# JuliaGaussianProcesses/ApproximateGPs.jl

Hardware: AMD Instinct MI355X
Metric: SVGP ELBO evals/sec at N=1e6, M=1024 (higher is better)
Workload: dtype f64

## Files before the change

### approximategps.jl_amd/csrc/device_common.hpp

```cpp
#pragma once
#include <hip/hip_runtime.h>
#include <type_traits>
#include <utility>

#include "diag.hpp"
#include <stdint.h>

#include <mutex>
#include <string>
#include <vector>

namespace svgp {

inline std::string& note_text() { static thread_local std::string s; return s; }
inline void leave_note(const std::string& s) {
  if (note_text().size() < 2048) note_text() += (note_text().empty() ? "" : "; ") + s;
}
inline std::string take_note() {
  std::string s;
  s.swap(note_text());
  return s;
}

inline void set_max_lds(const void* fn, hipFuncAttribute attr, int bytes) {
  struct Entry { const void* fn; int dev; int bytes; };
  static std::mutex mu;
  static std::vector<Entry> seen;
  int dev = 0;
  (void)hipGetDevice(&dev);
  std::lock_guard<std::mutex> g(mu);
  for (Entry& e : seen)
    if (e.fn == fn && e.dev == dev) {
      if (bytes <= e.bytes) return;
      if (hipFuncSetAttribute(fn, attr, bytes) == hipSuccess) e.bytes = bytes;
      else leave_note("hipFuncSetAttribute(" + std::to_string(bytes) + " bytes of LDS) failed");
      return;
    }
  const hipError_t err = hipFuncSetAttribute(fn, attr, bytes);
  if (err == hipSuccess) seen.push_back(Entry{fn, dev, bytes});
  else leave_note(std::string("hipFuncSetAttribute(") + std::to_string(bytes) + " bytes of LDS) failed: " + hipGetErrorString(err));
}

constexpr int kWave = 64;
constexpr int kThreads = 512;
constexpr int k256 = 256;
constexpr int kNB = 128;

template <typename T>
struct Mfma16;

template <>
struct Mfma16<double> {
  using acc_t = double __attribute__((ext_vector_type(4)));
  static __device__ __forceinline__ acc_t mma(double a, double b, acc_t c) {
    return __builtin_amdgcn_mfma_f64_16x16x4f64(a, b, c, 0, 0, 0);
  }
  static __device__ __forceinline__ int row(int lane, int r) { return (lane >> 4) + 4 * r; }
};

template <>
struct Mfma16<float> {
  using acc_t = float __attribute__((ext_vector_type(4)));
  static __device__ __forceinline__ acc_t mma(float a, float b, acc_t c) {
    return __builtin_amdgcn_mfma_f32_16x16x4f32(a, b, c, 0, 0, 0);
  }
  static __device__ __forceinline__ int row(int lane, int r) { return (lane >> 4) * 4 + r; }
};

template <typename T>
struct Vec16 {
  static constexpr int N = 16 / sizeof(T);
  using type = T __attribute__((ext_vector_type(16 / sizeof(T))));
};

enum : int { KSE = 0, KM32 = 1, KM52 = 2 };

__device__ __forceinline__ double kexp(double v) {
  const double n = rint(v * 1.4426950408889634074);
  double r = fma(n, -6.93147180369123816490e-01, v);
  r = fma(n, -1.90821492927058770002e-10, r);
  double p = 1.6059043836821613e-10;
  p = fma(p, r, 2.08767569878681e-09);
  p = fma(p, r, 2.505210838544172e-08);
  p = fma(p, r, 2.755731922398589e-07);
  p = fma(p, r, 2.7557319223985893e-06);
  p = fma(p, r, 2.48015873015873e-05);
  p = fma(p, r, 1.984126984126984e-04);
  p = fma(p, r, 1.3888888888888889e-03);
  p = fma(p, r, 8.333333333333333e-03);
  p = fma(p, r, 4.1666666666666664e-02);
  p = fma(p, r, 1.6666666666666666e-01);
  p = fma(p, r, 0.5);
  p = fma(p, r, 1.0);
  p = fma(p, r, 1.0);
  return ldexp(p, int(n));
}
__device__ __forceinline__ float kexp(float v) {
  const float hi = v * 1.44269504088896341f;
  const float lo = fmaf(v, 1.44269504088896341f, -hi) + v * 1.92596299112661746e-8f;
  const float e = __builtin_amdgcn_exp2f(hi);
  return fmaf(e, lo * 0.693147180559945309f, e);
}
__device__ __forceinline__ double kexp_tab(double v, const double* __restrict__ tab) {
  const double nd = rint(v * 92.332482616893658);
  const int n = int(nd);
  double r = fma(nd, -1.08304246932675596327e-02, v);
  r = fma(nd, -2.98158582698529328128e-12, r);
  const double t = tab[n & 63];
  double p = fma(r, 8.333333333333333e-03, 4.1666666666666664e-02);
  p = fma(p, r, 1.6666666666666666e-01);
  p = fma(p, r, 0.5);
  p = fma(p, r, 1.0);
  p *= r;
  return ldexp(fma(t, p, t), n >> 6);
}

__device__ __forceinline__ double ksqrt(double v) { return sqrt(v); }
__device__ __forceinline__ float ksqrt(float v) { return __builtin_amdgcn_sqrtf(v); }

template <typename T>
__device__ __forceinline__ T kappa(int family, T r2, T variance) {
  if (family == KSE) return variance * kexp(T(-0.5) * r2);
  T r = ksqrt(r2);
  if (family == KM32) {
    T s = T(1.7320508075688772935) * r;
    return variance * (T(1) + s) * kexp(-s);
  }
  T s = T(2.2360679774997896964) * r;
  return variance * (T(1) + s + T(5.0 / 3.0) * r2) * kexp(-s);
}

template <typename T>
__device__ __forceinline__ T kappa_2g(int family, T r2, T variance, T kval) {
  if (family == KSE) return -kval;
  T r = ksqrt(r2);
  if (family == KM32) {
    T s = T(1.7320508075688772935) * r;
    return (T(-3) * variance) * kexp(-s);
  }
  T s = T(2.2360679774997896964) * r;
  return (T(-5.0 / 3.0) * variance) * ((T(1) + s) * kexp(-s));
}

template <typename T, int NT, int BK, int NTHR = kThreads, int PAD = 16>
struct TileGemm {
  static constexpr int NB = kNB;
  static constexpr int WR = 2, WC = NTHR / 128;
  static constexpr int MI = NB / WR / 16;
  static constexpr int NJ = NT / WC / 16;
  static constexpr int PLD = NB + PAD;
  static constexpr int QLD = NT + PAD;
  static constexpr int VEC = Vec16<T>::N;
  using V = typename Vec16<T>::type;
  using acc_t = typename Mfma16<T>::acc_t;

  static constexpr int P_TPR = NB / VEC;
  static constexpr int P_RPP = NTHR / P_TPR;
  static constexpr int P_PASSES = BK / P_RPP;
  static constexpr int Q_TPR = NT / VEC;
  static constexpr int Q_RPP = NTHR / Q_TPR;
  static constexpr int Q_PASSES = (BK / Q_RPP) > 0 ? (BK / Q_RPP) : 1;
  static_assert(BK % P_RPP == 0, "BK must be a multiple of the P rows per pass");
  static_assert(BK % Q_RPP == 0 || Q_RPP % BK == 0, "BK and the Q rows per pass must divide one another");
  static constexpr bool Q_PARTIAL = Q_RPP > BK;

  static constexpr int P_TILE = BK * PLD;
  static constexpr int Q_TILE = BK * QLD;
  static constexpr int STAGE = P_TILE + Q_TILE;
  static constexpr size_t LDS_BYTES = 2 * size_t(STAGE) * sizeof(T);

  struct Acc {
    acc_t v[MI][NJ];
    __device__ __forceinline__ void zero() {
#pragma unroll
      for (int i = 0; i < MI; ++i)
#pragma unroll
        for (int j = 0; j < NJ; ++j) v[i][j] = acc_t{0, 0, 0, 0};
    }
  };

  struct PRegs { V v[P_PASSES]; };
  struct QRegs { V v[Q_PASSES]; };

  struct POff { uint32_t o[P_PASSES]; };
  struct QOff { uint32_t o[Q_PASSES]; };
  static __device__ __forceinline__ POff p_offsets(int64_t ld) {
    POff r;
    const int t = threadIdx.x;
    const int kk0 = t / P_TPR, c = (t % P_TPR) * VEC;
#pragma unroll
    for (int p = 0; p < P_PASSES; ++p) r.o[p] = uint32_t((int64_t(kk0 + p * P_RPP) * ld + c) * sizeof(T));
    return r;
  }
  static __device__ __forceinline__ QOff q_offsets(int64_t ld) {
    QOff r;
    const int t = threadIdx.x;
    const int kk0 = t / Q_TPR, c = (t % Q_TPR) * VEC;
#pragma unroll
    for (int p = 0; p < Q_PASSES; ++p) r.o[p] = uint32_t((int64_t(kk0 + p * Q_RPP) * ld + c) * sizeof(T));
    return r;
  }
  static __device__ __forceinline__ void load_p(PRegs& r, const T* __restrict__ src, const POff& off) {
    if constexpr (diag::ablate<1>) {
      asm volatile("" : "+v"(r.v[0]));
      return;
    }
    const char* base = reinterpret_cast<const char*>(src);
#pragma unroll
    for (int p = 0; p < P_PASSES; ++p) r.v[p] = *reinterpret_cast<const V*>(base + off.o[p]);
  }
  static __device__ __forceinline__ void store_p(const PRegs& r, T* __restrict__ Ps) {
    const int t = threadIdx.x;
    const int kk0 = t / P_TPR, c = (t % P_TPR) * VEC;
#pragma unroll
    for (int p = 0; p < P_PASSES; ++p) *reinterpret_cast<V*>(Ps + (kk0 + p * P_RPP) * PLD + c) = r.v[p];
  }
#ifndef SVGP_DMA_P
#define SVGP_DMA_P 1
#endif
#ifndef SVGP_DMA_ASM
#define SVGP_DMA_ASM 1
#endif
  static constexpr int NW = NTHR / 64;
  static constexpr bool kDmaP = SVGP_DMA_P && (NB * sizeof(T) == 1024) && (BK % NW == 0);
  static constexpr int D_ROWS = BK / NW;
  struct DOff { uint32_t o[D_ROWS]; };
  static __device__ __forceinline__ DOff d_offsets(int64_t ld) {
    DOff r;
    const int lane = threadIdx.x & 63, wave = threadIdx.x >> 6;
#pragma unroll
    for (int q = 0; q < D_ROWS; ++q) r.o[q] = uint32_t((int64_t(wave + q * NW) * ld + lane * VEC) * sizeof(T));
    return r;
  }
  static __device__ __forceinline__ void glds16(const void* sbase, uint32_t voff, const T* lds) {
#if SVGP_DMA_ASM
    const uint32_t l = uint32_t(uintptr_t((__attribute__((address_space(3))) T*)(lds)));
    asm volatile("s_mov_b32 m0, %0\n\tglobal_load_lds_dwordx4 %1, %2" ::"s"(l), "v"(voff), "s"(sbase) : "memory");
#else
    __builtin_amdgcn_global_load_lds((const __attribute__((address_space(1))) void*)(reinterpret_cast<const char*>(sbase) + voff),
                                     (__attribute__((address_space(3))) void*)(lds), 16, 0, 0);
#endif
  }
  static __device__ __forceinline__ void dma_p(const T* __restrict__ src, const DOff& off, T* __restrict__ Ps) {
    if constexpr (diag::ablate<1>) return;
    const int wv = __builtin_amdgcn_readfirstlane(int(threadIdx.x >> 6));
#pragma unroll
    for (int q = 0; q < D_ROWS; ++q) glds16(src, off.o[q], Ps + (wv + q * NW) * PLD);
  }
  static __device__ __forceinline__ void load_q(QRegs& r, const T* __restrict__ src, const QOff& off) {
    if constexpr (diag::ablate<2>) {
      asm volatile("" : "+v"(r.v[0]));
      return;
    }
    const char* base = reinterpret_cast<const char*>(src);
    if (Q_PARTIAL && int(threadIdx.x) >= BK * Q_TPR) return;
#pragma unroll
    for (int p = 0; p < Q_PASSES; ++p) r.v[p] = *reinterpret_cast<const V*>(base + off.o[p]);
  }
  static __device__ __forceinline__ void load_q_trans(QRegs& r, const T* __restrict__ src, int64_t ld) {
    const int t = threadIdx.x;
    const int kk0 = t / Q_TPR, c = (t % Q_TPR) * VEC;
#pragma unroll
    for (int p = 0; p < Q_PASSES; ++p)
#pragma unroll
      for (int e = 0; e < VEC; ++e) r.v[p][e] = src[int64_t(c + e) * ld + (kk0 + p * Q_RPP)];
  }
  static __device__ __forceinline__ void store_q(const QRegs& r, T* __restrict__ Qs) {
    const int t = threadIdx.x;
    const int kk0 = t / Q_TPR, c = (t % Q_TPR) * VEC;
    if (Q_PARTIAL && t >= BK * Q_TPR) return;
#pragma unroll
    for (int p = 0; p < Q_PASSES; ++p) *reinterpret_cast<V*>(Qs + (kk0 + p * Q_RPP) * QLD + c) = r.v[p];
  }
  static __device__ __forceinline__ void q_coord(int p, int& kk, int& c) {
    const int t = threadIdx.x;
    kk = t / Q_TPR + p * Q_RPP;
    c = (t % Q_TPR) * VEC;
  }

  struct Frag {
    T a[MI], b[NJ];
  };
  static __device__ __forceinline__ int wave_row() { return __builtin_amdgcn_readfirstlane(int(threadIdx.x >> 6)) / WC; }
  static __device__ __forceinline__ int frag_a_off() {
    const int lane = threadIdx.x & 63, wave = threadIdx.x >> 6;
    return (lane >> 4) * PLD + (wave / WC) * 16 + (lane & 15);
  }
  static __device__ __forceinline__ int frag_b_off() {
    const int lane = threadIdx.x & 63, wave = threadIdx.x >> 6;
    return (lane >> 4) * QLD + (wave % WC) * (NJ * 16) + (lane & 15);
  }
  template <int BUF, int KSLAB, int ILO = 0, int IHI = MI - 1>
  static __device__ __forceinline__ void load_frag(Frag& f, const T* __restrict__ fa, const T* __restrict__ fb) {
#pragma unroll
    for (int i = 0; i < MI; ++i)
      if (i >= ILO && i <= IHI) f.a[i] = fa[BUF * STAGE + KSLAB * 4 * PLD + i * 32];
    if (ILO <= IHI) {
#pragma unroll
      for (int j = 0; j < NJ; ++j) f.b[j] = fb[BUF * STAGE + KSLAB * 4 * QLD + j * 16];
    }
  }
  template <int ILO = 0, int IHI = MI - 1>
  static __device__ __forceinline__ void mma_frag(Acc& acc, const Frag& f) {
#pragma unroll
    for (int i = 0; i < MI; ++i)
      if (i >= ILO && i <= IHI) {
#pragma unroll
        for (int j = 0; j < NJ; ++j) acc.v[i][j] = Mfma16<T>::mma(f.a[i], f.b[j], acc.v[i][j]);
      }
  }

  static __device__ __forceinline__ int acc_row(int i, int r) {
    const int lane = threadIdx.x & 63, wave = threadIdx.x >> 6;
    return (2 * i + wave / WC) * 16 + Mfma16<T>::row(lane, r);
  }
  static __device__ __forceinline__ int acc_col(int j) {
    const int lane = threadIdx.x & 63, wave = threadIdx.x >> 6;
    return (wave % WC) * (NJ * 16) + j * 16 + (lane & 15);
  }

  static constexpr int kLoopPrologueBarriers = 1, kLoopClosingBarriers = 1;
  static constexpr int kAsyncPrologueBarriers = 1, kAsyncClosingBarriers = 1;
  static constexpr int loop_barrier_count(int nsteps) { return nsteps <= 0 ? 0 : kLoopPrologueBarriers + nsteps + kLoopClosingBarriers; }
  static constexpr int async_barrier_count(int nsteps) { return nsteps <= 0 ? 0 : kAsyncPrologueBarriers + (nsteps - 1) + kAsyncClosingBarriers; }

  template <int BUF, int ILO, int IHI, typename QLoad>
  static __device__ __forceinline__ void step(Acc& acc, Frag (&f)[2], PRegs& pr, QRegs& qr, const T* __restrict__ Pbase,
                                              int64_t pstride, const POff& poff, const DOff& doff, int t, int nsteps,
                                              QLoad& qload, T* __restrict__ smem, const T* __restrict__ fa,
                                              const T* __restrict__ fb) {
    constexpr int KS = BK / 4;
    static_assert(KS % 2 == 0, "the fragment ping-pong needs an even number of k-slabs per step");
    const bool more = (t + 1 < nsteps);
#pragma unroll
    for (int ks = 0; ks + 1 < KS; ++ks) {
      if (ks == 0) load_frag<BUF, 1, ILO, IHI>(f[1], fa, fb);
      if (ks == 1) load_frag<BUF, 2, ILO, IHI>(f[0], fa, fb);
      if (ks == 2) load_frag<BUF, 3, ILO, IHI>(f[1], fa, fb);
      if (ks == 3) load_frag<BUF, 4 < KS ? 4 : 0, ILO, IHI>(f[0], fa, fb);
      if (ks == 4) load_frag<BUF, 5 < KS ? 5 : 0, ILO, IHI>(f[1], fa, fb);
      if (ks == 5) load_frag<BUF, 6 < KS ? 6 : 0, ILO, IHI>(f[0], fa, fb);
      if (ks == 6) load_frag<BUF, 7 < KS ? 7 : 0, ILO, IHI>(f[1], fa, fb);
      mma_frag<ILO, IHI>(acc, f[ks & 1]);
    }
    if (more) {
      T* Pn = smem + (BUF ^ 1) * STAGE;
      if constexpr (!kDmaP) store_p(pr, Pn);
      store_q(qr, Pn + P_TILE);
    }
    __syncthreads();
    if (more) {
      load_frag<BUF ^ 1, 0>(f[0], fa, fb);
      if (t + 2 < nsteps) {
        if constexpr (kDmaP) {
          qload(t + 2, qr);
          dma_p(Pbase + int64_t(t + 2) * pstride, doff, smem + BUF * STAGE);
        } else {
          load_p(pr, Pbase + int64_t(t + 2) * pstride, poff);
          qload(t + 2, qr);
        }
      }
    }
    mma_frag<ILO, IHI>(acc, f[(KS - 1) & 1]);
  }

#define SVGP_DSTEP(B, LO, HI, TT) step<B, LO, HI>(acc, f, pr, qr, Pbase, pstride, poff, doff, (TT), nsteps, qload, smem, fa, fb)

  template <typename QLoad>
  static __device__ __forceinline__ void loop(Acc& acc, const T* __restrict__ Pbase, int64_t ldp, int nsteps,
                                              QLoad&& qload, T* __restrict__ smem) {
    loop_tri<0>(acc, Pbase, ldp, nsteps, qload, smem);
  }

  template <int TRI, typename QLoad>
  static __device__ __forceinline__ void loop_tri(Acc& acc, const T* __restrict__ Pbase, int64_t ldp, int nsteps,
                                                  QLoad&& qload, T* __restrict__ smem) {
    if (nsteps <= 0) return;
    static_assert(BK <= 32, "step() enumerates at most 8 k-slabs");
    constexpr int ND = NB / BK;
    static_assert(TRI == 0 || (ND == 8 && MI == 4), "triangular steps are written out for BK = 16, 128-row panels");
    const POff poff = p_offsets(ldp);
    const DOff doff = d_offsets(ldp);
    const int64_t pstride = int64_t(BK) * ldp;
    const T* fa = smem + frag_a_off();
    const T* fb = smem + P_TILE + frag_b_off();
    PRegs pr;
    QRegs qr;
    if constexpr (kDmaP) {
      qload(0, qr);
      dma_p(Pbase, doff, smem);
    } else {
      load_p(pr, Pbase, poff);
      qload(0, qr);
      store_p(pr, smem);
    }
    store_q(qr, smem + P_TILE);
    __syncthreads();
    if (nsteps > 1) {
      if constexpr (kDmaP) {
        qload(1, qr);
        dma_p(Pbase + pstride, doff, smem + STAGE);
      } else {
        load_p(pr, Pbase + pstride, poff);
        qload(1, qr);
      }
    }
    Frag f[2];
    load_frag<0, 0>(f[0], fa, fb);
    int t = 0;
    if (TRI < 0) {
      SVGP_DSTEP(0, 0, 0, 0); SVGP_DSTEP(1, 0, 0, 1); SVGP_DSTEP(0, 0, 1, 2); SVGP_DSTEP(1, 0, 1, 3);
      SVGP_DSTEP(0, 0, 2, 4); SVGP_DSTEP(1, 0, 2, 5); SVGP_DSTEP(0, 0, 3, 6); SVGP_DSTEP(1, 0, 3, 7);
      t = ND;
    }
    const int nreg = (TRI > 0) ? nsteps - ND : nsteps;
    for (; t + 1 < nreg; t += 2) {
      step<0, 0, MI - 1>(acc, f, pr, qr, Pbase, pstride, poff, doff, t, nsteps, qload, smem, fa, fb);
      step<1, 0, MI - 1>(acc, f, pr, qr, Pbase, pstride, poff, doff, t + 1, nsteps, qload, smem, fa, fb);
    }
    if (t < nreg) step<0, 0, MI - 1>(acc, f, pr, qr, Pbase, pstride, poff, doff, t, nsteps, qload, smem, fa, fb);
    if (TRI > 0) {
      SVGP_DSTEP(0, 0, 3, nreg + 0); SVGP_DSTEP(1, 0, 3, nreg + 1); SVGP_DSTEP(0, 1, 3, nreg + 2); SVGP_DSTEP(1, 1, 3, nreg + 3);
      SVGP_DSTEP(0, 2, 3, nreg + 4); SVGP_DSTEP(1, 2, 3, nreg + 5); SVGP_DSTEP(0, 3, 3, nreg + 6); SVGP_DSTEP(1, 3, 3, nreg + 7);
    }
    __syncthreads();
  }
#undef SVGP_DSTEP

  static constexpr bool kPairP = (NB * sizeof(T) == 512);
#ifndef SVGP_ASYNC_QUAD
#define SVGP_ASYNC_QUAD 1
#endif
  static constexpr bool kRowQ = (NT * sizeof(T) == 1024);
  static constexpr int QR = kRowQ ? 1 : ((NT * sizeof(T) == 256) ? 4 : 2);
  static constexpr bool kAsync = (SVGP_DMA_P != 0) && (NB * sizeof(T) == 1024 || kPairP) &&
                                 (NT * sizeof(T) == 512 || (SVGP_ASYNC_QUAD && NT * sizeof(T) == 256) || (kRowQ && NTHR == 512)) &&
                                 BK == 16 && (NTHR == 256 || (kRowQ && NTHR == 512)) && NJ % 2 == 0;
  static constexpr int NBUF = 3;
  static constexpr int QPP = kRowQ ? QLD : QR * NT;
  static constexpr int QA_TILE = (BK / QR) * QPP;
  static constexpr int QSLAB = (4 / QR) * QPP;
  static constexpr int PPP = 2 * NB;
  static constexpr int PA_TILE = kPairP ? (BK / 2) * PPP : P_TILE;
  static constexpr int DQ = (BK / QR) / NW;
  static constexpr int DP = kPairP ? (BK / 2) / NW : BK / NW;
  static constexpr int DMA_PER_TILE = DP + DQ;
  static constexpr size_t ASYNC_LDS_BYTES = size_t(NBUF) * (PA_TILE + QA_TILE) * sizeof(T);
  static constexpr int W_TILE = 256 / int(sizeof(T));
  static constexpr size_t ASYNC_W_LDS_BYTES = ASYNC_LDS_BYTES + size_t(NBUF) * 256;
  static constexpr size_t MAX_LDS_BYTES = (kAsync && ASYNC_LDS_BYTES > LDS_BYTES) ? ASYNC_LDS_BYTES : LDS_BYTES;

  struct AOff { uint32_t p[DP]; uint32_t q[DQ]; };
  static __device__ __forceinline__ AOff a_offsets(int64_t ldp, int64_t ldq) {
    AOff r;
    const int lane = threadIdx.x & 63, wave = threadIdx.x >> 6;
    const int row = lane >> 5, slot = (lane & 31) * VEC;
#pragma unroll
    for (int q = 0; q < DP; ++q) {
      if constexpr (kPairP) r.p[q] = uint32_t((int64_t((wave + q * NW) * 2 + row) * ldp + (slot ^ (row * 16))) * sizeof(T));
      else r.p[q] = uint32_t((int64_t(wave + q * NW) * ldp + lane * VEC) * sizeof(T));
    }
    constexpr int LPR = 64 / QR;
    const int qrow = lane / LPR, qslot = (lane % LPR) * VEC;
#pragma unroll
    for (int q = 0; q < DQ; ++q)
      r.q[q] = uint32_t((int64_t((wave + q * NW) * QR + qrow) * ldq + (qslot ^ (qrow * 16))) * sizeof(T));
    return r;
  }
  static __device__ __forceinline__ int wave_index() { return __builtin_amdgcn_readfirstlane(int(threadIdx.x >> 6)); }
  static __device__ __forceinline__ void dma_tile(const T* __restrict__ psrc, const T* __restrict__ qsrc, const AOff& off,
                                                  T* __restrict__ Pb, T* __restrict__ Qb) {
    const int wv = wave_index();
// ... 364 lines not shown
```

### approximategps.jl_amd/csrc/strip.hip

```cpp
#define SVGP_DIAG_TU_STRIP
#include "device_common.hpp"
#include "kernels.hpp"
#include "knobs.hpp"
#include "lik.hpp"

#ifndef SVGP_ASYNC
#define SVGP_ASYNC 1
#endif
#ifndef SVGP_TRI
#define SVGP_TRI 3
#endif

#include <cstdlib>
#include <type_traits>

namespace svgp {

namespace {

#ifndef SVGP_PREGEN_EXPTAB
#define SVGP_PREGEN_EXPTAB 1
#endif
template <typename T, int NT, int NTHR, int F, int DL>
__device__ __forceinline__ void pregen_mfma(const T* __restrict__ xs, const T* __restrict__ zs, int d, int64_t Mp, int64_t M,
                                            double variance_d, T* __restrict__ work, const double* __restrict__ exptab = nullptr) {
  constexpr int KS = DL / 4, JT = NT / 16, NW = NTHR / 64;
  constexpr bool XREG = (DL <= 16);
  using M16 = Mfma16<T>;
  using acc_t = typename M16::acc_t;
  const int lane = threadIdx.x & 63, wave = threadIdx.x >> 6, l15 = lane & 15, g = lane >> 4;
  const T variance = T(variance_d);
  const T c1 = (F == KSE) ? T(-0.5) : T(1);
  const T c0 = (F == KSE) ? T(log(variance_d)) : T(0);
  const T ascale = (F == KSE) ? T(1) : T(-2);
  T xb[XREG ? JT : 1][XREG ? KS : 1], xn[JT];
  const T* __restrict__ xl = xs + g * NT + l15;
#pragma unroll
  for (int jt = 0; jt < JT; ++jt) {
    T s = T(0);
#pragma unroll
    for (int q = 0; q < KS; ++q) {
      const T v = xl[(4 * q) * NT + jt * 16];
      if constexpr (XREG) xb[jt][q] = v;
      s = fma(v, v, s);
    }
    s += __shfl_xor(s, 16);
    s += __shfl_xor(s, 32);
    xn[jt] = fma(c1, s, c0);
  }
  for (int kb = wave; kb < int(Mp / 16); kb += NW) {
    const int64_t k0 = int64_t(kb) * 16;
    const bool inside = __builtin_amdgcn_readfirstlane(int(k0 + 16 <= M)) != 0;
    T za[KS];
    T s = T(0);
#pragma unroll
    for (int q = 0; q < KS; ++q) {
      const int f = 4 * q + g;
      const T v = (f < d) ? zs[int64_t(f) * Mp + k0 + l15] : T(0);
      za[q] = ascale * v;
      s = fma(v, v, s);
    }
    s += __shfl_xor(s, 16);
    s += __shfl_xor(s, 32);
    s *= c1;
    T zn[4];
#pragma unroll
    for (int r = 0; r < 4; ++r) zn[r] = __shfl(s, M16::row(lane, r));
#pragma unroll
    for (int jt = 0; jt < JT; ++jt) {
      acc_t acc;
#pragma unroll
      for (int r = 0; r < 4; ++r) acc[r] = xn[jt] + zn[r];
      if constexpr (XREG) {
#pragma unroll
        for (int q = 0; q < KS; ++q) acc = M16::mma(za[q], xb[jt][q], acc);
      } else {
        acc_t acc2 = {0, 0, 0, 0};
        __builtin_amdgcn_sched_barrier(0);
#pragma unroll
        for (int q = 0; q < KS; q += 2) {
          acc = M16::mma(za[q], xl[(4 * q) * NT + jt * 16], acc);
          acc2 = M16::mma(za[q + 1], xl[(4 * q + 4) * NT + jt * 16], acc2);
        }
#pragma unroll
        for (int r = 0; r < 4; ++r) acc[r] += acc2[r];
      }
      T out[4];
#pragma unroll
      for (int r = 0; r < 4; ++r) {
        const T v = acc[r];
        if constexpr (SVGP_PREGEN_EXPTAB && F == KSE && sizeof(T) == 8) out[r] = T(kexp_tab(double(v > c0 ? c0 : v), exptab));
        else out[r] = (F == KSE) ? kexp(v > c0 ? c0 : v) : kappa<T>(F, v < T(0) ? T(0) : v, variance);
      }
      if (inside) {
#pragma unroll
        for (int r = 0; r < 4; ++r) work[(k0 + M16::row(lane, r)) * NT + jt * 16 + l15] = out[r];
      } else {
#pragma unroll
        for (int r = 0; r < 4; ++r) {
          const int64_t k = k0 + M16::row(lane, r);
          work[k * NT + jt * 16 + l15] = (k < M) ? out[r] : T(0);
        }
        asm volatile("" ::: "memory");
      }
    }
  }
}


template <typename G, typename T, int NT, int NTHR>
__device__ __forceinline__ void store_tile_point_major(const typename G::Acc& acc, T* __restrict__ smem, T* __restrict__ out,
                                                       int64_t c0, int64_t Mp, int row0) {
  constexpr int HC = NT < 64 ? NT : 64, RS = G::NB + (sizeof(T) == 8 ? 4 : 8), VEC = G::VEC, CPR = G::NB / VEC;
  using V = typename G::V;
  static_assert(size_t(HC) * RS * sizeof(T) <= ((SVGP_ASYNC && G::kAsync) ? G::ASYNC_LDS_BYTES : G::LDS_BYTES),
                "the transposition tile must fit the staging buffers");
#pragma unroll
  for (int p = 0; p < NT / HC; ++p) {
#pragma unroll
    for (int j = 0; j < G::NJ; ++j) {
      const int col = G::acc_col(j);
      if (col / HC == p) {
#pragma unroll
        for (int i = 0; i < G::MI; ++i)
#pragma unroll
          for (int r = 0; r < 4; ++r) smem[(col % HC) * RS + G::acc_row(i, r)] = acc.v[i][j][r];
      }
    }
    __syncthreads();
    for (int e = threadIdx.x; e < HC * CPR; e += NTHR) {
      const int col = e / CPR, rv = (e % CPR) * VEC;
      *reinterpret_cast<V*>(out + (c0 + p * HC + col) * Mp + row0 + rv) = *reinterpret_cast<const V*>(smem + col * RS + rv);
    }
    __syncthreads();
  }
}

#ifndef SVGP_STRIP_PRIO
#define SVGP_STRIP_PRIO 1
#endif
template <bool ON>
__device__ __forceinline__ void strip_prio(int strips_done) {
  if constexpr (ON && SVGP_STRIP_PRIO != 0) {
    if ((strips_done + (blockIdx.x >= gridDim.x / 2 ? 1 : 0)) & 1) __builtin_amdgcn_s_setprio(0);
    else __builtin_amdgcn_s_setprio(1);
  }
}

struct PointGrads { double e, gmu, gv, gs2; };
__device__ __noinline__ PointGrads strip_point_grads(LikParams lp, double mu, double v, double yv, double scale) {
  double a = 0.0, b = 0.0, gs2 = 0.0;
  expected_loglik_grad_point(lp, mu, v, yv, a, b, gs2);
  PointGrads r;
  r.e = expected_loglik_point(lp, mu, v, yv, log(lp.sigma2));
  r.gmu = a * scale;
  r.gv = b * scale;
  r.gs2 = gs2 * scale;
  return r;
}

template <typename T, int NT, int BK, int NTHR, int MINW = 2, int PAD = 16, bool GRAD = false, bool BIGD = false, bool SEG = false>
__global__ void __launch_bounds__(NTHR, MINW) strip_kernel(StripArgs a, int64_t nstrips) {
  using G = TileGemm<T, NT, BK, NTHR, PAD>;
  using Acc = typename G::Acc;
  using QRegs = typename G::QRegs;
  constexpr int NB = G::NB, MI = G::MI, NJ = G::NJ, VEC = G::VEC;

  extern __shared__ __attribute__((aligned(16))) unsigned char smem_raw[];
  T* smem = reinterpret_cast<T*>(smem_raw);
  T* xs = smem;
  const int pre_dl = BIGD ? (a.kp.d <= 32 ? 32 : 64) : (a.kp.d <= 8 ? 8 : a.kp.d <= 16 ? 16 : 0);
  const int dl = pre_dl ? pre_dl : a.kp.d;

  const T* __restrict__ Tm = static_cast<const T*>(a.T);
  const T* __restrict__ U = static_cast<const T*>(a.U);
  const T* __restrict__ zs = static_cast<const T*>(a.zs);
  const T* __restrict__ mp = static_cast<const T*>(a.mp);
  const T* __restrict__ x = static_cast<const T*>(a.x);
  const T* __restrict__ invl = static_cast<const T*>(a.kp.invl);
  const int64_t Mp = a.Mp, M = a.M;
  const int d = a.kp.d, family = a.kp.family;
  const T variance = T(a.kp.variance);
  const int nP = int(Mp / NB);
  T* __restrict__ work = static_cast<T*>(a.work) + int64_t(blockIdx.x) * Mp * NT;
  T* __restrict__ workK = (GRAD && !diag::ablate<256>) ? static_cast<T*>(a.work) + (int64_t(gridDim.x) + blockIdx.x) * Mp * NT : work;
  const int tid = threadIdx.x, lane = tid & 63;
  const typename G::QOff qoff = G::q_offsets(NT);

  __shared__ unsigned next_strip;
#if SVGP_PREGEN_EXPTAB
  __shared__ double s_exptab[64];
  if (sizeof(T) == 8 && threadIdx.x < 64) s_exptab[threadIdx.x] = exp2(double(threadIdx.x) * 0.015625);
  const double* exptab = s_exptab;
#else
  const double* exptab = nullptr;
#endif
  SVGP_SSTAMP_KERNEL_BEGIN();
  [[maybe_unused]] int prio_strips = 0;
  [[maybe_unused]] int part = 0, nsplit = 1;
  if constexpr (SEG) {
    if (a.seg_split > 1) { nsplit = a.seg_split; part = int(blockIdx.x / nstrips); }
  }
  for (int64_t strip = (nsplit > 1) ? int64_t(blockIdx.x % nstrips) : int64_t(blockIdx.x); strip < nstrips;) {
    if constexpr (SEG) {
      work = static_cast<T*>(a.work) + strip * Mp * NT;
      workK = GRAD ? static_cast<T*>(a.work) + (nstrips + strip) * Mp * NT : work;
    }
    SVGP_SSTAMP_STRIP_BEGIN();
    SVGP_SSTAMP(0);
    strip_prio<GRAD && !SEG>(prio_strips++);
    const int64_t c0 = strip * NT;
    if constexpr (SEG) { if (tid == 0) next_strip = unsigned(strip + gridDim.x); }
    else if (tid == 0) next_strip = gridDim.x + atomicAdd(a.counter, 1u);
    const int64_t last = a.off + a.len - 1;
    const bool do_pregen = !SEG || (a.seg_flags & kSegPregen);
    if (do_pregen)
    for (int e = tid; e < dl * NT; e += NTHR) {
      const int f = e / NT, c = e % NT;
      int64_t g = a.off + c0 + c;
      g = g > last ? last : g;
      xs[e] = (f < d) ? x[int64_t(f) * a.ldx + g] * invl[f] : T(0);
    }
    __syncthreads();
    if (do_pregen) {
      auto pregen = [&](auto fam) {
        constexpr int F = decltype(fam)::value;
        using V = typename G::V;
        constexpr int CPR = NT / VEC;
        for (int e = tid; e < int(Mp) * CPR; e += NTHR) {
          const int k = e / CPR, c = (e % CPR) * VEC;
          T r2[VEC];
#pragma unroll
          for (int q = 0; q < VEC; ++q) r2[q] = T(0);
#pragma unroll 8
          for (int f = 0; f < d; ++f) {
            const T zf = zs[int64_t(f) * Mp + k];
            const V xf = *reinterpret_cast<const V*>(xs + f * NT + c);
#pragma unroll
            for (int q = 0; q < VEC; ++q) {
              const T df = xf[q] - zf;
              r2[q] = fma(df, df, r2[q]);
            }
          }
          V out;
#pragma unroll
          for (int q = 0; q < VEC; ++q) out[q] = (k < M) ? kappa<T>(F, r2[q], variance) : T(0);
          *reinterpret_cast<V*>(workK + int64_t(k) * NT + c) = out;
        }
      };
      if constexpr (BIGD) {
        if (pre_dl == 32) {
          if (family == KSE) pregen_mfma<T, NT, NTHR, KSE, 32>(xs, zs, d, Mp, M, a.kp.variance, workK, exptab);
          else if (family == KM32) pregen_mfma<T, NT, NTHR, KM32, 32>(xs, zs, d, Mp, M, a.kp.variance, workK);
          else pregen_mfma<T, NT, NTHR, KM52, 32>(xs, zs, d, Mp, M, a.kp.variance, workK);
        } else {
          if (family == KSE) pregen_mfma<T, NT, NTHR, KSE, 64>(xs, zs, d, Mp, M, a.kp.variance, workK, exptab);
          else if (family == KM32) pregen_mfma<T, NT, NTHR, KM32, 64>(xs, zs, d, Mp, M, a.kp.variance, workK);
          else pregen_mfma<T, NT, NTHR, KM52, 64>(xs, zs, d, Mp, M, a.kp.variance, workK);
        }
      } else if (pre_dl == 8) {
        if (family == KSE) pregen_mfma<T, NT, NTHR, KSE, 8>(xs, zs, d, Mp, M, a.kp.variance, workK, exptab);
        else if (family == KM32) pregen_mfma<T, NT, NTHR, KM32, 8>(xs, zs, d, Mp, M, a.kp.variance, workK);
        else pregen_mfma<T, NT, NTHR, KM52, 8>(xs, zs, d, Mp, M, a.kp.variance, workK);
      } else if (pre_dl == 16) {
        if (family == KSE) pregen_mfma<T, NT, NTHR, KSE, 16>(xs, zs, d, Mp, M, a.kp.variance, workK, exptab);
        else if (family == KM32) pregen_mfma<T, NT, NTHR, KM32, 16>(xs, zs, d, Mp, M, a.kp.variance, workK);
        else pregen_mfma<T, NT, NTHR, KM52, 16>(xs, zs, d, Mp, M, a.kp.variance, workK);
      } else if (family == KSE) pregen(std::integral_constant<int, KSE>{});
      else if (family == KM32) pregen(std::integral_constant<int, KM32>{});
      else pregen(std::integral_constant<int, KM52>{});
      __syncthreads();
    }

    double sA[NJ], sM[NJ], sC[NJ];
#pragma unroll
    for (int j = 0; j < NJ; ++j) sA[j] = sM[j] = sC[j] = 0.0;
    int I_lo = 0, I_hi = nP;
    if constexpr (SEG) {
      I_lo = a.seg_lo;
      I_hi = a.seg_hi;
      if ((a.seg_flags & kSegLoad) && part == 0) {
        const double* __restrict__ st = a.seg_state + (strip * NTHR + tid) * (2 * NJ);
#pragma unroll
        for (int j = 0; j < NJ; ++j) { sA[j] = st[j]; sM[j] = st[NJ + j]; }
      }
    }

    SVGP_SSTAMP(1);
    for (int I = I_lo; I < I_hi; ++I) {
      SVGP_SSTAMP(2 + 3 * I);
      Acc acc;
      acc.zero();
      const int tK = I * (NB / BK);
      if constexpr (SVGP_ASYNC && G::kAsync) {
        auto qsrc = [&](int t) { return (t < tK ? work : workK) + int64_t(t) * BK * NT; };
        G::template loop_tri_async<(SVGP_TRI & 1) ? 1 : 0>(acc, Tm + int64_t(I) * NB, Mp, (I + 1) * (NB / BK), qsrc, smem);
      } else {
        auto qload = [&](int t, QRegs& r) { G::load_q(r, (t < tK ? work : workK) + int64_t(t) * BK * NT, qoff); };
        G::template loop_tri<(BK == 16 && (SVGP_TRI & 1)) ? 1 : 0>(acc, Tm + int64_t(I) * NB, Mp, (I + 1) * (NB / BK), qload, smem);
      }

      SVGP_SSTAMP(3 + 3 * I);
#pragma unroll
      for (int i = 0; i < MI; ++i) {
#pragma unroll
        for (int r = 0; r < 4; ++r) {
          const int row = I * NB + G::acc_row(i, r);
          const double mr = double(mp[row]);
#pragma unroll
          for (int j = 0; j < NJ; ++j) {
            const T val = acc.v[i][j][r];
            const int col = G::acc_col(j);
            if constexpr (!diag::ablate<4>) work[int64_t(row) * NT + col] = val;
            if (a.A_out) static_cast<T*>(a.A_out)[int64_t(row) * a.lda + c0 + col] = val;
            if constexpr (!GRAD) {
              if (a.At_out) static_cast<T*>(a.At_out)[(c0 + col) * Mp + row] = val;
            }
            if constexpr (!diag::ablate<16>) {
              const double dv = double(val);
              if constexpr (!GRAD) sA[j] = fma(dv, dv, sA[j]);
              sM[j] = fma(dv, mr, sM[j]);
            } else {
              sA[j] += double(val) + mr;
            }
          }
        }
      }
      if constexpr (GRAD && !diag::ablate<32>) store_tile_point_major<G, T, NT, NTHR>(acc, smem, static_cast<T*>(a.At_out), c0, Mp, I * NB);
      __syncthreads();
      SVGP_SSTAMP(4 + 3 * I);
    }

    if constexpr (SEG) {
      if (a.seg_flags & kSegStore) {
        double* __restrict__ st = a.seg_state + (strip * NTHR + tid) * (2 * NJ);
#pragma unroll
        for (int j = 0; j < NJ; ++j) { st[j] = sA[j]; st[NJ + j] = sM[j]; }
      }
      if (!(a.seg_flags & kSegPhase2)) {
        strip = next_strip;
        __syncthreads();
        continue;
      }
    }
    if constexpr (!GRAD)
    for (int J = SEG ? part : 0; J < nP; J += (SEG ? nsplit : 1)) {
      SVGP_SSTAMP(60 + 2 * J);
      Acc acc;
      acc.zero();
      const T* wq = work + int64_t(J) * NB * NT;
      if constexpr (SVGP_ASYNC && G::kAsync) {
        auto qsrc = [&](int t) { return wq + int64_t(t) * BK * NT; };
        G::template loop_tri_async<(SVGP_TRI & 2) ? -1 : 0>(acc, U + int64_t(J) * NB + int64_t(J) * NB * Mp, Mp, (nP - J) * (NB / BK), qsrc,
                                                            smem);
      } else {
        auto qload = [&](int t, QRegs& r) { G::load_q(r, wq + int64_t(t) * BK * NT, qoff); };
        G::template loop_tri<(BK == 16 && (SVGP_TRI & 2)) ? -1 : 0>(acc, U + int64_t(J) * NB + int64_t(J) * NB * Mp, Mp, (nP - J) * (NB / BK), qload,
                                                   smem);
      }
      SVGP_SSTAMP(61 + 2 * J);
#pragma unroll
      for (int i = 0; i < MI; ++i)
#pragma unroll
        for (int r = 0; r < 4; ++r)
#pragma unroll
          for (int j = 0; j < NJ; ++j) {
            const T val = acc.v[i][j][r];
            if (a.C_out) static_cast<T*>(a.C_out)[int64_t(J * NB + G::acc_row(i, r)) * a.lda + c0 + G::acc_col(j)] = val;
            if (a.Ct_out) static_cast<T*>(a.Ct_out)[(c0 + G::acc_col(j)) * Mp + J * NB + G::acc_row(i, r)] = val;
            const double dv = double(val);
            sC[j] = fma(dv, dv, sC[j]);
          }
    }

    if constexpr (GRAD) {
      const T* __restrict__ Rm = static_cast<const T*>(a.R);
      T* __restrict__ Pt = static_cast<T*>(a.Pt_out);
      int p3_lo = 0, p3_hi = nP;
      if constexpr (SEG) { p3_lo = (part * nP) / nsplit; p3_hi = ((part + 1) * nP) / nsplit; }
      for (int I = p3_lo; I < p3_hi; ++I) {
        SVGP_SSTAMP(26 + 4 * I);
        Acc acc;
        acc.zero();
        if constexpr (SVGP_ASYNC && G::kAsync) {
          auto qsrc = [&](int t) { return work + int64_t(t) * BK * NT; };
          G::template loop_tri_async<0>(acc, Rm + int64_t(I) * NB, Mp, nP * (NB / BK), qsrc, smem);
        } else {
          auto qload = [&](int t, QRegs& r) { G::load_q(r, work + int64_t(t) * BK * NT, qoff); };
          G::template loop_tri<0>(acc, Rm + int64_t(I) * NB, Mp, nP * (NB / BK), qload, smem);
        }
        SVGP_SSTAMP(27 + 4 * I);
        if constexpr (!diag::ablate<128>) {
#pragma unroll
          for (int i = 0; i < MI; ++i)
#pragma unroll
            for (int r = 0; r < 4; ++r) {
              const int64_t row = int64_t(I) * NB + G::acc_row(i, r);
#pragma unroll
              for (int j = 0; j < NJ; ++j) sC[j] = fma(double(acc.v[i][j][r]), double(workK[row * NT + G::acc_col(j)]), sC[j]);
            }
        } else {
#pragma unroll
          for (int j = 0; j < NJ; ++j) sC[j] += double(acc.v[0][j][0]);
        }
        SVGP_SSTAMP(28 + 4 * I);
        if constexpr (!diag::ablate<64>) store_tile_point_major<G, T, NT, NTHR>(acc, smem, Pt, c0, Mp, I * NB);
        else if (acc.v[0][0][0] == T(12345.678)) Pt[c0] = acc.v[0][0][0];
        SVGP_SSTAMP(29 + 4 * I);
      }
    }

    SVGP_SSTAMP(100);
    double* red = reinterpret_cast<double*>(smem_raw);
#pragma unroll
    for (int j = 0; j < NJ; ++j) {
      double va = sA[j], vm = sM[j], vc = sC[j];
      va += __shfl_xor(va, 16); va += __shfl_xor(va, 32);
      vm += __shfl_xor(vm, 16); vm += __shfl_xor(vm, 32);
      vc += __shfl_xor(vc, 16); vc += __shfl_xor(vc, 32);
      if ((lane >> 4) == 0) {
        const int wr = (tid >> 6) / G::WC;
        const int col = G::acc_col(j);
        red[(0 * G::WR + wr) * NT + col] = va;
        red[(1 * G::WR + wr) * NT + col] = vm;
        red[(2 * G::WR + wr) * NT + col] = vc;
      }
    }
    __syncthreads();
    {
      bool split_done = false;
      if constexpr (SEG) {
        if (nsplit > 1) {
          __shared__ int s_last_part;
          if (tid < NT) {
            double qa = 0, qm = 0, qc = 0;
#pragma unroll
            for (int w = 0; w < G::WR; ++w) {
              qa += red[(0 * G::WR + w) * NT + tid];
              qm += red[(1 * G::WR + w) * NT + tid];
              qc += red[(2 * G::WR + w) * NT + tid];
            }
            double* __restrict__ pp = a.seg_part + ((int64_t(part) * nstrips + strip) * 3) * NT;
            pp[tid] = qa;
            pp[NT + tid] = qm;
            pp[2 * NT + tid] = qc;
          }
          __threadfence();
          __syncthreads();
          if (tid == 0) s_last_part = (__hip_atomic_fetch_add(&a.seg_cnt[strip], 1u, __ATOMIC_ACQ_REL, __HIP_MEMORY_SCOPE_AGENT) == unsigned(nsplit - 1));
          __syncthreads();
          if (s_last_part) {
            __threadfence();
            if (tid < NT && c0 + tid < a.len) {
              double qa = 0, qm = 0, qc = 0;
              for (int q = 0; q < nsplit; ++q) {
                const double* __restrict__ pp = a.seg_part + ((int64_t(q) * nstrips + strip) * 3) * NT;
                qa += __builtin_nontemporal_load(pp + tid);
                qm += __builtin_nontemporal_load(pp + NT + tid);
                qc += __builtin_nontemporal_load(pp + 2 * NT + tid);
              }
              const double mc = a.mux ? a.mean_const + double(static_cast<const T*>(a.mux)[c0 + tid]) : a.mean_const;
              a.mom_mu[c0 + tid] = mc + qm;
              a.mom_var[c0 + tid] = a.kp.variance - qa + qc;
            }
          }
          __syncthreads();
          split_done = true;
        }
      }
      if (!split_done) {
      if (tid < NT && c0 + tid < a.len) {
        double qa = 0, qm = 0, qc = 0;
#pragma unroll
        for (int w = 0; w < G::WR; ++w) {
          qa += red[(0 * G::WR + w) * NT + tid];
          qm += red[(1 * G::WR + w) * NT + tid];
          qc += red[(2 * G::WR + w) * NT + tid];
        }
        const double mc = a.mux ? a.mean_const + double(static_cast<const T*>(a.mux)[c0 + tid]) : a.mean_const;
        a.mom_mu[c0 + tid] = mc + qm;
        a.mom_var[c0 + tid] = a.kp.variance - qa + qc;
      }
      __syncthreads();
      }
    }
    strip = next_strip;
    __syncthreads();
    SVGP_SSTAMP(101);
  }
  SVGP_SSTAMP_KERNEL_END();
}

template <typename T, int NT, int BK, int NTHR, int MINW = 2, int PAD = 16, bool BIGD = false>
__global__ void __launch_bounds__(NTHR, MINW) trsm_pm_kernel(StripArgs a, int64_t nstrips) {
  using G = TileGemm<T, NT, BK, NTHR, PAD>;
  using Acc = typename G::Acc;
  using QRegs = typename G::QRegs;
  constexpr int NB = G::NB, MI = G::MI, NJ = G::NJ;

  extern __shared__ __attribute__((aligned(16))) unsigned char smem_raw[];
  T* smem = reinterpret_cast<T*>(smem_raw);
  T* xs = smem;
  const int pre_dl = BIGD ? (a.kp.d <= 32 ? 32 : 64) : (a.kp.d <= 8 ? 8 : 16);
  const T* __restrict__ Tm = static_cast<const T*>(a.T);
  const T* __restrict__ zs = static_cast<const T*>(a.zs);
  const T* __restrict__ x = static_cast<const T*>(a.x);
  const T* __restrict__ invl = static_cast<const T*>(a.kp.invl);
  const int64_t Mp = a.Mp, M = a.M;
  const int d = a.kp.d, family = a.kp.family;
  const int nP = int(Mp / NB);
  T* __restrict__ work = static_cast<T*>(a.work) + int64_t(blockIdx.x) * Mp * NT;
  const int tid = threadIdx.x, lane = tid & 63;
  [[maybe_unused]] const typename G::QOff qoff = G::q_offsets(NT);
// ... 729 lines not shown
```

Measured before the change: 29.25.

## Software-pipeline KSE pregen exp with next block's distances; lean strip epilogues

Adds a pipelined path for the f64 squared-exponential pregen: the next block's Z features are prefetched and its MFMA distance tile is computed while the current tile's table-based exponentials are evaluated in batches. A vectorised kexp_tab_n helper lets the compiler interleave several independent exp evaluations. It also adds lean epilogues for the forward, non-segmented strip kernel that skip per-element checks of the optional A/At/C/Ct output pointers and use precomputed row/column offsets. Register pressure rises from the extra in-flight accumulators and prefetched values, which may reduce occupancy.

Result: faster. 29.66, median of 6 (+1.4%).

```diff
diff --git a/approximategps.jl_amd/csrc/device_common.hpp b/approximategps.jl_amd/csrc/device_common.hpp
--- a/approximategps.jl_amd/csrc/device_common.hpp
+++ b/approximategps.jl_amd/csrc/device_common.hpp
@@ -101,18 +101,39 @@
   const float e = __builtin_amdgcn_exp2f(hi);
   return fmaf(e, lo * 0.693147180559945309f, e);
 }
+template <int N>
+__device__ __forceinline__ void kexp_tab_n(const double (&v)[N], double (&out)[N], const double* __restrict__ tab) {
+  double nd[N], r[N], t[N], p[N];
+  int n[N];
+#pragma unroll
+  for (int e = 0; e < N; ++e) nd[e] = rint(v[e] * 92.332482616893658);
+#pragma unroll
+  for (int e = 0; e < N; ++e) n[e] = int(nd[e]);
+#pragma unroll
+  for (int e = 0; e < N; ++e) r[e] = fma(nd[e], -1.08304246932675596327e-02, v[e]);
+#pragma unroll
+  for (int e = 0; e < N; ++e) r[e] = fma(nd[e], -2.98158582698529328128e-12, r[e]);
+#pragma unroll
+  for (int e = 0; e < N; ++e) t[e] = tab[n[e] & 63];
+#pragma unroll
+  for (int e = 0; e < N; ++e) p[e] = fma(r[e], 8.333333333333333e-03, 4.1666666666666664e-02);
+#pragma unroll
+  for (int e = 0; e < N; ++e) p[e] = fma(p[e], r[e], 1.6666666666666666e-01);
+#pragma unroll
+  for (int e = 0; e < N; ++e) p[e] = fma(p[e], r[e], 0.5);
+#pragma unroll
+  for (int e = 0; e < N; ++e) p[e] = fma(p[e], r[e], 1.0);
+#pragma unroll
+  for (int e = 0; e < N; ++e) p[e] *= r[e];
+#pragma unroll
+  for (int e = 0; e < N; ++e) out[e] = ldexp(fma(t[e], p[e], t[e]), n[e] >> 6);
+}
+
 __device__ __forceinline__ double kexp_tab(double v, const double* __restrict__ tab) {
-  const double nd = rint(v * 92.332482616893658);
-  const int n = int(nd);
-  double r = fma(nd, -1.08304246932675596327e-02, v);
-  r = fma(nd, -2.98158582698529328128e-12, r);
-  const double t = tab[n & 63];
-  double p = fma(r, 8.333333333333333e-03, 4.1666666666666664e-02);
-  p = fma(p, r, 1.6666666666666666e-01);
-  p = fma(p, r, 0.5);
-  p = fma(p, r, 1.0);
-  p *= r;
-  return ldexp(fma(t, p, t), n >> 6);
+  const double a[1] = {v};
+  double o[1];
+  kexp_tab_n<1>(a, o, tab);
+  return o[0];
 }
 
 __device__ __forceinline__ double ksqrt(double v) { return sqrt(v); }
@@ -318,6 +339,8 @@
     const int lane = threadIdx.x & 63, wave = threadIdx.x >> 6;
     return (wave % WC) * (NJ * 16) + j * 16 + (lane & 15);
   }
+  static constexpr int acc_row_rel(int i, int r) { return 32 * i + (sizeof(T) == 8 ? 4 * r : r); }
+  static constexpr int acc_col_rel(int j) { return 16 * j; }
 
   static constexpr int kLoopPrologueBarriers = 1, kLoopClosingBarriers = 1;
   static constexpr int kAsyncPrologueBarriers = 1, kAsyncClosingBarriers = 1;
diff --git a/approximategps.jl_amd/csrc/strip.hip b/approximategps.jl_amd/csrc/strip.hip
--- a/approximategps.jl_amd/csrc/strip.hip
+++ b/approximategps.jl_amd/csrc/strip.hip
@@ -21,7 +21,10 @@
 #ifndef SVGP_PREGEN_EXPTAB
 #define SVGP_PREGEN_EXPTAB 1
 #endif
-template <typename T, int NT, int NTHR, int F, int DL>
+#ifndef SVGP_PREGEN_PIPE
+#define SVGP_PREGEN_PIPE 1
+#endif
+template <typename T, int NT, int NTHR, int F, int DL, bool PIPE = false>
 __device__ __forceinline__ void pregen_mfma(const T* __restrict__ xs, const T* __restrict__ zs, int d, int64_t Mp, int64_t M,
                                             double variance_d, T* __restrict__ work, const double* __restrict__ exptab = nullptr) {
   constexpr int KS = DL / 4, JT = NT / 16, NW = NTHR / 64;
@@ -48,6 +51,83 @@
     s += __shfl_xor(s, 32);
     xn[jt] = fma(c1, s, c0);
   }
+  if constexpr (XREG && PIPE && F == KSE && sizeof(T) == 8 && SVGP_PREGEN_EXPTAB != 0 && SVGP_PREGEN_PIPE != 0) {
+    constexpr int EG = JT >= 2 ? 2 : 1;
+    static_assert(JT % EG == 0, "whole groups");
+    const int nblk = int(Mp / 16);
+    auto zfetch = [&](int kb, T (&zv)[KS]) {
+#pragma unroll
+      for (int q = 0; q < KS; ++q) {
+        const int f = 4 * q + g;
+        zv[q] = zs[int64_t(f < d ? f : 0) * Mp + int64_t(kb) * 16 + l15];
+      }
+    };
+    acc_t acc[JT];
+    auto distances = [&](const T (&zv)[KS]) {
+      T za[KS];
+      T s = T(0);
+#pragma unroll
+      for (int q = 0; q < KS; ++q) {
+        const T v = (4 * q + g < d) ? zv[q] : T(0);
+        za[q] = ascale * v;
+        s = fma(v, v, s);
+      }
+      s += __shfl_xor(s, 16);
+      s += __shfl_xor(s, 32);
+      s *= c1;
+      T zn[4];
+#pragma unroll
+      for (int r = 0; r < 4; ++r) zn[r] = __shfl(s, M16::row(lane, r));
+#pragma unroll
+      for (int jt = 0; jt < JT; ++jt)
+#pragma unroll
+        for (int r = 0; r < 4; ++r) acc[jt][r] = xn[jt] + zn[r];
+#pragma unroll
+      for (int q = 0; q < KS; ++q)
+#pragma unroll
+        for (int jt = 0; jt < JT; ++jt) acc[jt] = M16::mma(za[q], xb[jt][q], acc[jt]);
+    };
+    T zv[KS];
+    zfetch(wave < nblk ? wave : 0, zv);
+    distances(zv);
+    for (int kb = wave; kb < nblk; kb += NW) {
+      const int64_t k0 = int64_t(kb) * 16;
+      const bool inside = __builtin_amdgcn_readfirstlane(int(k0 + 16 <= M)) != 0;
+      zfetch(kb + NW < nblk ? kb + NW : kb, zv);
+      double out[JT * 4];
+#pragma unroll
+      for (int g0 = 0; g0 < JT; g0 += EG) {
+        double v[EG * 4], o[EG * 4];
+#pragma unroll
+        for (int e = 0; e < EG * 4; ++e) {
+          const double w = acc[g0 + e / 4][e % 4];
+          v[e] = w > c0 ? c0 : w;
+        }
+        kexp_tab_n<EG * 4>(v, o, exptab);
+#pragma unroll
+        for (int e = 0; e < EG * 4; ++e) out[g0 * 4 + e] = o[e];
+        __builtin_amdgcn_sched_barrier(0);
+      }
+      distances(zv);
+      __builtin_amdgcn_sched_barrier(0);
+      if (inside) {
+#pragma unroll
+        for (int jt = 0; jt < JT; ++jt)
+#pragma unroll
+          for (int r = 0; r < 4; ++r) work[(k0 + M16::row(lane, r)) * NT + jt * 16 + l15] = out[jt * 4 + r];
+      } else {
+#pragma unroll
+        for (int jt = 0; jt < JT; ++jt)
+#pragma unroll
+          for (int r = 0; r < 4; ++r) {
+            const int64_t k = k0 + M16::row(lane, r);
+            work[k * NT + jt * 16 + l15] = (k < M) ? out[jt * 4 + r] : T(0);
+          }
+        asm volatile("" ::: "memory");
+      }
+    }
+    return;
+  }
   for (int kb = wave; kb < int(Mp / 16); kb += NW) {
     const int64_t k0 = int64_t(kb) * 16;
     const bool inside = __builtin_amdgcn_readfirstlane(int(k0 + 16 <= M)) != 0;
@@ -138,6 +218,9 @@
 
 #ifndef SVGP_STRIP_PRIO
 #define SVGP_STRIP_PRIO 1
+#endif
+#ifndef SVGP_EPI_LEAN
+#define SVGP_EPI_LEAN 1
 #endif
 template <bool ON>
 __device__ __forceinline__ void strip_prio(int strips_done) {
@@ -186,6 +269,9 @@
   T* __restrict__ workK = (GRAD && !diag::ablate<256>) ? static_cast<T*>(a.work) + (int64_t(gridDim.x) + blockIdx.x) * Mp * NT : work;
   const int tid = threadIdx.x, lane = tid & 63;
   const typename G::QOff qoff = G::q_offsets(NT);
+  constexpr bool kLeanEpi = SVGP_EPI_LEAN != 0 && !GRAD && !SEG && sizeof(T) == 8;
+  [[maybe_unused]] const uint32_t epi_woff = uint32_t((G::acc_row(0, 0) * NT + G::acc_col(0)) * int(sizeof(T)));
+  [[maybe_unused]] const uint32_t epi_moff = uint32_t(G::acc_row(0, 0) * int(sizeof(T)));
 
   __shared__ unsigned next_strip;
 #if SVGP_PREGEN_EXPTAB
@@ -259,11 +345,11 @@
           else pregen_mfma<T, NT, NTHR, KM52, 64>(xs, zs, d, Mp, M, a.kp.variance, workK);
         }
       } else if (pre_dl == 8) {
-        if (family == KSE) pregen_mfma<T, NT, NTHR, KSE, 8>(xs, zs, d, Mp, M, a.kp.variance, workK, exptab);
+        if (family == KSE) pregen_mfma<T, NT, NTHR, KSE, 8, !GRAD && !SEG>(xs, zs, d, Mp, M, a.kp.variance, workK, exptab);
         else if (family == KM32) pregen_mfma<T, NT, NTHR, KM32, 8>(xs, zs, d, Mp, M, a.kp.variance, workK);
         else pregen_mfma<T, NT, NTHR, KM52, 8>(xs, zs, d, Mp, M, a.kp.variance, workK);
       } else if (pre_dl == 16) {
-        if (family == KSE) pregen_mfma<T, NT, NTHR, KSE, 16>(xs, zs, d, Mp, M, a.kp.variance, workK, exptab);
+        if (family == KSE) pregen_mfma<T, NT, NTHR, KSE, 16, !GRAD && !SEG>(xs, zs, d, Mp, M, a.kp.variance, workK, exptab);
         else if (family == KM32) pregen_mfma<T, NT, NTHR, KM32, 16>(xs, zs, d, Mp, M, a.kp.variance, workK);
         else pregen_mfma<T, NT, NTHR, KM52, 16>(xs, zs, d, Mp, M, a.kp.variance, workK);
       } else if (family == KSE) pregen(std::integral_constant<int, KSE>{});
@@ -301,6 +387,51 @@
       }
 
       SVGP_SSTAMP(3 + 3 * I);
+      if (kLeanEpi && a.A_out == nullptr && a.At_out == nullptr) {
+        T* wI = work + int64_t(I) * NB * NT;
+        const T* mpI = mp + I * NB;
+        double mr[MI][4];
+#pragma unroll
+        for (int i = 0; i < MI; ++i)
+#pragma unroll
+          for (int r = 0; r < 4; ++r)
+            mr[i][r] = double(*reinterpret_cast<const T*>(reinterpret_cast<const char*>(mpI + G::acc_row_rel(i, r)) + epi_moff));
+        if constexpr (!diag::ablate<16>) {
+#pragma unroll
+          for (int i = 0; i < MI; ++i)
+#pragma unroll
+            for (int r = 0; r < 4; ++r)
+#pragma unroll
+              for (int j = 0; j < NJ; ++j) {
+                const double dv = double(acc.v[i][j][r]);
+                sA[j] = fma(dv, dv, sA[j]);
+              }
+#pragma unroll
+          for (int i = 0; i < MI; ++i)
+#pragma unroll
+            for (int r = 0; r < 4; ++r)
+#pragma unroll
+              for (int j = 0; j < NJ; ++j) sM[j] = fma(double(acc.v[i][j][r]), mr[i][r], sM[j]);
+        } else {
+#pragma unroll
+          for (int i = 0; i < MI; ++i)
+#pragma unroll
+            for (int r = 0; r < 4; ++r)
+#pragma unroll
+              for (int j = 0; j < NJ; ++j) sA[j] += double(acc.v[i][j][r]) + mr[i][r];
+        }
+        __builtin_amdgcn_sched_barrier(0);
+        if constexpr (!diag::ablate<4>) {
+#pragma unroll
+          for (int i = 0; i < MI; ++i)
+#pragma unroll
+            for (int r = 0; r < 4; ++r) {
+              T* wr = reinterpret_cast<T*>(reinterpret_cast<char*>(wI + G::acc_row_rel(i, r) * NT) + epi_woff);
+#pragma unroll
+              for (int j = 0; j < NJ; ++j) wr[G::acc_col_rel(j)] = acc.v[i][j][r];
+            }
+        }
+      } else {
 #pragma unroll
       for (int i = 0; i < MI; ++i) {
 #pragma unroll
@@ -326,6 +457,7 @@
           }
         }
       }
+      }
       if constexpr (GRAD && !diag::ablate<32>) store_tile_point_major<G, T, NT, NTHR>(acc, smem, static_cast<T*>(a.At_out), c0, Mp, I * NB);
       __syncthreads();
       SVGP_SSTAMP(4 + 3 * I);
@@ -359,6 +491,17 @@
                                                    smem);
       }
       SVGP_SSTAMP(61 + 2 * J);
+      if (kLeanEpi && a.C_out == nullptr && a.Ct_out == nullptr) {
+#pragma unroll
+        for (int i = 0; i < MI; ++i)
+#pragma unroll
+          for (int r = 0; r < 4; ++r)
+#pragma unroll
+            for (int j = 0; j < NJ; ++j) {
+              const double dv = double(acc.v[i][j][r]);
+              sC[j] = fma(dv, dv, sC[j]);
+            }
+      } else
 #pragma unroll
       for (int i = 0; i < MI; ++i)
 #pragma unroll
```
